# ska-sa/katsdpsigproc

Hardware: AMD Instinct MI355X
Metric: visibility samples/s (baselines x channels) through full RFI flagger (higher is better)
Workload: dtype f32 amplitude / f64 deviations

## Files before the change

### include/katsdpsigproc_hip.h

```cpp
#ifndef KATSDPSIGPROC_HIP_H
#define KATSDPSIGPROC_HIP_H

#include <stddef.h>
#include <stdint.h>

#ifdef __cplusplus
extern "C" {
#endif

#define KSP_ABI_VERSION 5

#define KSP_FLAGS_NONE 0
#define KSP_FLAGS_CHANNEL 1
#define KSP_FLAGS_FULL 2

#define KSP_THRESHOLD_SIMPLE 0
#define KSP_THRESHOLD_SUM 1

#define KSP_MAX_WINDOWS 8

typedef struct ksp_device_props {
    char name[256];
    char arch[64];
    int32_t compute_units;
// ... 31 lines not shown
int ksp_memcpy_async(int device, void *dst, const void *src, size_t bytes, int kind,
                     void *stream);
int ksp_memcpy_rect_async(int device, void *dst, size_t dst_origin, const size_t dst_strides[3],
                          const void *src, size_t src_origin, const size_t src_strides[3],
                          const size_t shape[3], int ndim, int kind, void *stream);
int ksp_memset_async(int device, void *ptr, int value, size_t bytes, void *stream);


int ksp_transpose(int device, void *stream, void *dst, const void *src, int in_rows, int in_cols,
                  int out_stride, int in_stride, int elem_size);

int ksp_percentile5_float(int device, void *stream, const void *in, float *out, int rows,
                          int in_stride, int out_stride, int first_col, int n_cols,
                          int is_amplitude);

int ksp_maskedsum_float(int device, void *stream, const void *in, const float *mask, void *out,
                        int in_stride, int n_rows, int n_cols, int use_amplitudes);

int ksp_background_median_filter(int device, void *stream, const void *in, float *out,
                                 const uint8_t *flags, int channels, int baselines, int stride,
                                 int flags_stride, int width, int is_amplitude, int flags_mode,
                                 int csplit);

int ksp_background_median_filter_geometry(int channels, int baselines, int width, int csplit,
                                          int *seg_len, int *n_segs);

int ksp_madnz_t(int device, void *stream, const float *in, float *noise, int channels,
                int baselines, int stride);

int ksp_madnz(int device, void *stream, const float *in, float *noise, int channels,
              int baselines, int stride);

int ksp_threshold_simple(int device, void *stream, const float *deviations, const float *noise,
                         uint8_t *flags, int rows, int cols, int stride, float n_sigma,
                         int flag_value, int transposed);

int ksp_threshold_sum(int device, void *stream, const float *deviations, const float *noise,
                      uint8_t *flags, int channels, int baselines, int stride, float n_sigma,
                      const float *scales, int n_windows, int flag_value, int vt);

int ksp_threshold_sum_cm(int device, void *stream, const float *deviations, const float *noise,
                         uint8_t *flags, int channels, int baselines, int stride, float n_sigma,
                         const float *scales, int n_windows, int flag_value);

int ksp_flagger_fused(int device, void *stream, const void *vis, const uint8_t *in_flags,
                      uint8_t *flags, float *deviations, float *noise, int channels,
                      int baselines, int vis_stride, int in_flags_stride, int flags_stride,
                      int dev_stride, int width, int is_amplitude, int flags_mode,
                      int threshold_kind, double n_sigma, const double *scales64, int n_windows,
                      int flag_value, void *workspace);

int ksp_flagger_fused_profile(void *start_event, void *stop_event);

int ksp_flagger_fused_supported(int channels, int width, int n_windows);

#define KSP_FUSED_PATH_STRIP 1
#define KSP_FUSED_PATH_LONG 2
#define KSP_FUSED_PATH_RING 4
int ksp_flagger_fused_last_path(void);

int ksp_flagger_fused_ring_mode(int mode);

int ksp_selftest_sqrt12(int device, void *stream, float *out, int n);
int ksp_selftest_abs(int device, void *stream, const float *re, const float *im, float *out,
                     int n);

int ksp_selftest_rank(int device, void *stream, const float *data, int *out, int n, int m);
int ksp_selftest_minmax(int device, void *stream, const float *data, float *out, int n);
int ksp_selftest_median_non_zero(int device, void *stream, const float *data, float *out,
                                 int n);

int ksp_rtc_compile(int device, const char *source, const char *const *options, int n_options,
                    void **module_out, char *log, size_t log_capacity);
int ksp_module_get_function(int device, void *module, const char *name, void **function_out);
int ksp_module_unload(int device, void *module);
int ksp_launch_function(int device, void *stream, void *function, const unsigned *grid,
                        const unsigned *block, unsigned shared_bytes, void **kernel_params);

#define KSP_FFT_R2C 0x2a
#define KSP_FFT_C2R 0x2c
#define KSP_FFT_C2C 0x29
#define KSP_FFT_D2Z 0x6a
#define KSP_FFT_Z2D 0x6c
#define KSP_FFT_Z2Z 0x69
int ksp_fft_plan_create(int device, int rank, const long long *n, const long long *inembed,
                        long long idist, const long long *onembed, long long odist, int type,
                        long long batch, void **plan_out, size_t *work_size);
int ksp_fft_plan_destroy(int device, void *plan);
int ksp_fft_exec(int device, void *stream, void *plan, int type, void *src, void *dest,
                 void *work_area, int inverse);

#define KSP_TDF_MAX_TIME 4096
#define KSP_TDF_MAX_FREQ 65536
#define KSP_TDF_MAX_WINDOWS 32
#define KSP_TDF_MAX_CHUNKS 512
#define KSP_TDF_MAX_RADIUS 2047
typedef struct ksp_twodflag_params {
    int n_time, n_freq, average_freq, is_amplitude;
    int n_windows_time, n_windows_freq;
    int windows_time[KSP_TDF_MAX_WINDOWS], windows_freq[KSP_TDF_MAX_WINDOWS];
    double tf_time[KSP_TDF_MAX_WINDOWS], tf_freq[KSP_TDF_MAX_WINDOWS];
    int n_chunks;
    int chunk_ends[KSP_TDF_MAX_CHUNKS + 1];
    int background_iterations, time_extend, freq_extend;
    double spike_width_time, spike_width_freq;
    double threshold_scale, reject_scale, flag_all_time_frac, flag_all_freq_frac;
} ksp_twodflag_params;
int ksp_twodflag_workspace(const ksp_twodflag_params *params, int batch, size_t *bytes);
typedef struct ksp_twodflag_offsets {
    size_t spec_flags, spec_background, spec_residual, spec_st;
    size_t flags, background, residual, time_flags, freq_flags, combined;
    size_t row_flags, row_all, col_all;
} ksp_twodflag_offsets;
int ksp_twodflag_layout(const ksp_twodflag_params *params, int batch, ksp_twodflag_offsets *out);
int ksp_twodflag(int device, void *stream, const void *data, const uint8_t *in_flags,
// ... 113 lines not shown
```

### katsdpsigproc_amd/_lib.py

```python

import contextlib
import ctypes
import os
import sys
from ctypes import POINTER, byref, c_char_p, c_double, c_float, c_int, c_int32, c_int64, c_size_t
from ctypes import c_void_p

_HERE = os.path.dirname(os.path.abspath(__file__))
LIB_PATH = os.path.join(_HERE, "_native", "libkatsdpsigproc_hip.so")
ABI_VERSION = 5

FUSED_PATH_STRIP = 1
FUSED_PATH_LONG = 2
FUSED_PATH_RING = 4

_lib = None


class DeviceProps(ctypes.Structure):

    _fields_ = [
        ("name", ctypes.c_char * 256),
        ("arch", ctypes.c_char * 64),
        ("compute_units", c_int32),
# ... 17 lines not shown

    _fields_ = [
        ("n_time", c_int), ("n_freq", c_int), ("average_freq", c_int), ("is_amplitude", c_int),
        ("n_windows_time", c_int), ("n_windows_freq", c_int),
        ("windows_time", c_int * TDF_MAX_WINDOWS), ("windows_freq", c_int * TDF_MAX_WINDOWS),
        ("tf_time", c_double * TDF_MAX_WINDOWS), ("tf_freq", c_double * TDF_MAX_WINDOWS),
        ("n_chunks", c_int), ("chunk_ends", c_int * (TDF_MAX_CHUNKS + 1)),
        ("background_iterations", c_int), ("time_extend", c_int), ("freq_extend", c_int),
        ("spike_width_time", c_double), ("spike_width_freq", c_double),
        ("threshold_scale", c_double), ("reject_scale", c_double),
        ("flag_all_time_frac", c_double), ("flag_all_freq_frac", c_double),
    ]


class TwodflagOffsets(ctypes.Structure):

    _fields_ = [(name, c_size_t) for name in (
        "spec_flags", "spec_background", "spec_residual", "spec_st", "flags", "background",
        "residual", "time_flags", "freq_flags", "combined", "row_flags", "row_all", "col_all",
    )]


SIGNATURES = {
    "ksp_device_count": [POINTER(c_int)],
    "ksp_device_get_props": [c_int, POINTER(DeviceProps)],
    "ksp_malloc": [c_int, c_size_t, POINTER(c_void_p)],
    "ksp_free": [c_int, c_void_p],
    "ksp_host_alloc": [c_size_t, POINTER(c_void_p)],
    "ksp_host_free": [c_void_p],
    "ksp_stream_create": [c_int, POINTER(c_void_p)],
    "ksp_stream_destroy": [c_int, c_void_p],
    "ksp_stream_synchronize": [c_int, c_void_p],
    "ksp_event_create": [c_int, POINTER(c_void_p)],
    "ksp_event_create_ordering": [c_int, POINTER(c_void_p)],
    "ksp_event_destroy": [c_int, c_void_p],
    "ksp_event_record": [c_int, c_void_p, c_void_p],
    "ksp_event_synchronize": [c_int, c_void_p],
    "ksp_event_elapsed_ms": [c_int, c_void_p, c_void_p, POINTER(c_float)],
    "ksp_stream_wait_event": [c_int, c_void_p, c_void_p],
    "ksp_memcpy_async": [c_int, c_void_p, c_void_p, c_size_t, c_int, c_void_p],
    "ksp_memcpy_rect_async": [
        c_int, c_void_p, c_size_t, POINTER(c_size_t), c_void_p, c_size_t, POINTER(c_size_t),
        POINTER(c_size_t), c_int, c_int, c_void_p,
    ],
    "ksp_memset_async": [c_int, c_void_p, c_int, c_size_t, c_void_p],
    "ksp_transpose": [c_int, c_void_p, c_void_p, c_void_p, c_int, c_int, c_int, c_int, c_int],
    "ksp_percentile5_float": [
        c_int, c_void_p, c_void_p, c_void_p, c_int, c_int, c_int, c_int, c_int, c_int
    ],
    "ksp_maskedsum_float": [
        c_int, c_void_p, c_void_p, c_void_p, c_void_p, c_int, c_int, c_int, c_int
    ],
    "ksp_flagger_fused_profile": [c_void_p, c_void_p],
    "ksp_selftest_sqrt12": [c_int, c_void_p, c_void_p, c_int],
    "ksp_selftest_abs": [c_int, c_void_p, c_void_p, c_void_p, c_void_p, c_int],
    "ksp_selftest_rank": [c_int, c_void_p, c_void_p, c_void_p, c_int, c_int],
    "ksp_selftest_minmax": [c_int, c_void_p, c_void_p, c_void_p, c_int],
    "ksp_selftest_median_non_zero": [c_int, c_void_p, c_void_p, c_void_p, c_int],
    "ksp_background_median_filter": [
        c_int, c_void_p, c_void_p, c_void_p, c_void_p, c_int, c_int, c_int, c_int, c_int, c_int,
        c_int, c_int,
    ],
    "ksp_background_median_filter_geometry": [
        c_int, c_int, c_int, c_int, POINTER(c_int), POINTER(c_int)
    ],
    "ksp_madnz_t": [c_int, c_void_p, c_void_p, c_void_p, c_int, c_int, c_int],
    "ksp_madnz": [c_int, c_void_p, c_void_p, c_void_p, c_int, c_int, c_int],
    "ksp_threshold_simple": [
        c_int, c_void_p, c_void_p, c_void_p, c_void_p, c_int, c_int, c_int, c_float, c_int, c_int
    ],
    "ksp_threshold_sum": [
        c_int, c_void_p, c_void_p, c_void_p, c_void_p, c_int, c_int, c_int, c_float,
        POINTER(c_float), c_int, c_int, c_int,
    ],
    "ksp_threshold_sum_cm": [
        c_int, c_void_p, c_void_p, c_void_p, c_void_p, c_int, c_int, c_int, c_float,
        POINTER(c_float), c_int, c_int,
    ],
    "ksp_flagger_fused": [
        c_int, c_void_p, c_void_p, c_void_p, c_void_p, c_void_p, c_void_p, c_int, c_int, c_int,
        c_int, c_int, c_int, c_int, c_int, c_int, c_int, c_double, POINTER(c_double), c_int,
        c_int, c_void_p,
    ],
    "ksp_flagger_fused_supported": [c_int, c_int, c_int],
    "ksp_flagger_fused_last_path": [],
    "ksp_flagger_fused_ring_mode": [c_int],
    "ksp_rtc_compile": [
        c_int, c_char_p, POINTER(c_char_p), c_int, POINTER(c_void_p), c_char_p, c_size_t
    ],
    "ksp_module_get_function": [c_int, c_void_p, c_char_p, POINTER(c_void_p)],
    "ksp_module_unload": [c_int, c_void_p],
    "ksp_fft_plan_create": [
        c_int, c_int, POINTER(ctypes.c_longlong), POINTER(ctypes.c_longlong), ctypes.c_longlong,
        POINTER(ctypes.c_longlong), ctypes.c_longlong, c_int, ctypes.c_longlong,
        POINTER(c_void_p), POINTER(c_size_t),
    ],
    "ksp_fft_plan_destroy": [c_int, c_void_p],
    "ksp_fft_exec": [c_int, c_void_p, c_void_p, c_int, c_void_p, c_void_p, c_void_p, c_int],
    "ksp_twodflag_workspace": [POINTER(TwodflagParams), c_int, POINTER(c_size_t)],
    "ksp_twodflag_layout": [POINTER(TwodflagParams), c_int, POINTER(TwodflagOffsets)],
    "ksp_twodflag": [
        c_int, c_void_p, c_void_p, c_void_p, c_void_p, c_int, ctypes.c_longlong, ctypes.c_longlong,
        c_int, c_int, POINTER(TwodflagParams), c_void_p, c_size_t,
    ],
    "ksp_masked_filter_workspace": [
        c_int, c_int, c_int, c_int, c_int, c_int, c_int, POINTER(c_size_t),
# ... 150 lines not shown
```

### katsdpsigproc_amd/csrc/flagger_fused.hip

```cpp
#include "flagger_fused_kernel.h"

static thread_local hipEvent_t g_prof_start = nullptr, g_prof_stop = nullptr;
static thread_local int g_last_path = 0;

__global__ __launch_bounds__(256) void fused_zero_rows_kernel(uint8_t *__restrict__ base, int rows,
                                                              int cols, size_t stride, int pieces)
{
    const size_t gid = (size_t)blockIdx.x * 256 + threadIdx.x;
    const size_t row = gid / (unsigned)pieces;
    if (row >= (size_t)rows) return;
    const int k = (int)(gid - row * (unsigned)pieces);
    const uintptr_t begin = (uintptr_t)base + row * stride, end = begin + (uintptr_t)cols;
    const uintptr_t piece = (begin & ~(uintptr_t)15) + 16 * (uintptr_t)k;
    if (piece >= end) return;
    if (piece >= begin && piece + 16 <= end) {
        *(uint4 *)piece = make_uint4(0u, 0u, 0u, 0u);
    } else {
        const uintptr_t lo = piece > begin ? piece : begin;
        const uintptr_t hi = piece + 16 < end ? piece + 16 : end;
        for (uintptr_t a = lo; a < hi; a++) *(uint8_t *)a = 0;
    }
}

hipError_t fused_zero_flags(const FusedParams &p, hipStream_t s)
{
    if (p.flags_stride == p.baselines)
        return hipMemsetAsync(p.flags, 0, (size_t)p.channels * p.baselines, s);
    const int pieces = (p.baselines + 15) / 16 + 1;
    const size_t lanes = (size_t)p.channels * pieces;
    hipLaunchKernelGGL(fused_zero_rows_kernel, dim3((unsigned)((lanes + 255) / 256)), dim3(256), 0, s,
                       p.flags, p.channels, p.baselines, (size_t)p.flags_stride, pieces);
    return hipGetLastError();
}

extern "C" int ksp_flagger_fused_profile(void *start_event, void *stop_event)
{
    KSP_REQUIRE((start_event == nullptr) == (stop_event == nullptr), "need both events or none");
    g_prof_start = (hipEvent_t)start_event;
    g_prof_stop = (hipEvent_t)stop_event;
    return 0;
}

extern "C" int ksp_flagger_fused_last_path(void) { return g_last_path; }

static thread_local int g_ring_mode = 2;
static int ring_mode()
{
    if (g_ring_mode == 2) {
        const char *e = getenv("KSP_FUSED_RING");
        g_ring_mode = e == nullptr ? 0 : (e[0] == '1' ? 1 : -1);
    }
    return g_ring_mode;
}
extern "C" int ksp_flagger_fused_ring_mode(int mode)
{
    const int before = ring_mode();
    if (mode >= -1 && mode <= 1) g_ring_mode = mode;
    return before;
}

extern "C" int ksp_flagger_fused_supported(int channels, int width, int n_windows)
{
    if (n_windows < 1 || n_windows > KSP_MAX_WINDOWS) return 0;
    if (channels > 4096) return n_windows <= 4 && ksp_fused_long_supported(channels, width);
    return channels >= 1 && width >= 3 && width <= 31 && (width & 1);
}

static int check_fused_args(const void *vis, const uint8_t *in_flags, const uint8_t *flags,
                            const float *deviations, int channels, int baselines, int vis_stride,
                            int in_flags_stride, int flags_stride, int dev_stride, int width,
                            int flags_mode, int threshold_kind, const double *scales64,
                            int &n_windows)
{
    KSP_REQUIRE(vis != nullptr && flags != nullptr, "NULL buffer");
    KSP_REQUIRE(channels >= 1 && baselines >= 0, "bad shape");
    KSP_REQUIRE(vis_stride >= baselines && flags_stride >= baselines, "stride smaller than row");
    KSP_REQUIRE(deviations == nullptr || dev_stride >= baselines, "bad dev_stride");
    KSP_REQUIRE(flags_mode >= KSP_FLAGS_NONE && flags_mode <= KSP_FLAGS_FULL, "bad flags_mode");
    KSP_REQUIRE(flags_mode == KSP_FLAGS_NONE || in_flags != nullptr, "in_flags is NULL");
    KSP_REQUIRE(flags_mode != KSP_FLAGS_FULL || in_flags_stride >= baselines, "bad in_flags_stride");
    KSP_REQUIRE(threshold_kind == KSP_THRESHOLD_SIMPLE || threshold_kind == KSP_THRESHOLD_SUM,
                "bad threshold_kind");
    KSP_REQUIRE(threshold_kind == KSP_THRESHOLD_SIMPLE || scales64 != nullptr, "scales64 is NULL");
    if (threshold_kind == KSP_THRESHOLD_SIMPLE && n_windows < 1) n_windows = 1;
    if (!ksp_flagger_fused_supported(channels, width, n_windows)) {
        ksp_set_error("ksp_flagger_fused: unsupported configuration (channels=%d width=%d "
                      "n_windows=%d); use the per-stage kernels", channels, width, n_windows);
        return (int)hipErrorNotSupported;
    }
    KSP_REQUIRE((vis_stride & 1) == 0, "vis_stride must be even");
    KSP_REQUIRE(((uintptr_t)vis & 15) == 0, "vis must be 16-byte aligned");
    return 0;
}

static void set_schedule(FusedParams &p, bool have_workspace)
{
// ... 46 lines not shown
    FusedParams t = p;
    t.vis = (const float2 *)p.vis + first;
    t.flags = p.flags + first;
    if (p.noise != nullptr) t.noise = p.noise + first;
    t.baselines = count;
    set_schedule(t, false);
    return t;
}

struct FusedPath {
    int bits, lanes, tail;
};

static FusedPath choose_path(const FusedParams &p, int width, int n_cu, int mode)
{
    const bool want_ring = mode != 0 ? mode > 0 : p.baselines / 8 >= 4 * n_cu;
    if (want_ring && width == 13 && ksp_ring_supported(p, width)) {
        const int tail = p.baselines % 8;
        return {KSP_FUSED_PATH_RING | (tail != 0 ? KSP_FUSED_PATH_STRIP : 0), 64, tail};
    }
    if (p.channels > 4096) return {KSP_FUSED_PATH_LONG, 64, 0};
    const bool wide = p.threshold_kind == KSP_THRESHOLD_SUM && p.n_windows > 4;
    if (width != 13 || wide || p.channels > 64 * 16) return {KSP_FUSED_PATH_STRIP, 64, 0};
    return {KSP_FUSED_PATH_STRIP, p.channels <= 64 * 4 ? 4 : 16, 0};
}

static int launch_strip(int lanes, int width, int device, hipStream_t s, const FusedParams &p,
                        hipEvent_t ev0, hipEvent_t ev1)
{
    if (width == 13) {
        if (lanes == 64) return launch_fused<64, 13>(device, s, p, ev0, ev1);
        if (lanes == 4) return launch_fused<4, 13>(device, s, p, ev0, ev1);
        return launch_fused<16, 13>(device, s, p, ev0, ev1);
    }
    int rc = 0;
    if (ksp_dispatch_exact<3, 5, 7, 9, 11, 15, 17, 19, 21, 23, 25, 27, 29, 31>(width, [&](auto W) {
            rc = ksp_fused_launch_width<W()>(device, s, p, ev0, ev1);
        }))
        return rc;
    ksp_set_error("fused flagger: width %d is not compiled here", width);
    return (int)hipErrorInvalidValue;
}

extern "C" int ksp_flagger_fused(int device, void *stream, const void *vis,
                                 const uint8_t *in_flags, uint8_t *flags, float *deviations,
                                 float *noise, int channels, int baselines, int vis_stride,
                                 int in_flags_stride, int flags_stride, int dev_stride, int width,
                                 int is_amplitude, int flags_mode, int threshold_kind,
                                 double n_sigma, const double *scales64, int n_windows,
                                 int flag_value, void *workspace)
{
    const hipEvent_t ev0 = g_prof_start, ev1 = g_prof_stop;
    g_prof_start = g_prof_stop = nullptr;
    g_last_path = 0;
    int rc = check_fused_args(vis, in_flags, flags, deviations, channels, baselines, vis_stride,
                              in_flags_stride, flags_stride, dev_stride, width, flags_mode,
                              threshold_kind, scales64, n_windows);
    if (rc != 0 || baselines == 0) return rc;
    KSP_CHECK(hipSetDevice(device));
    static KspPerDevice<int> cus;
    int n_cu = cus.get(device);
    if (n_cu == 0) {
        KSP_CHECK(hipDeviceGetAttribute(&n_cu, hipDeviceAttributeMultiprocessorCount, device));
        cus.set(device, n_cu);
    }
    const FusedParams p = make_params(vis, in_flags, flags, deviations, noise, channels, baselines,
                                      vis_stride, in_flags_stride, flags_stride, dev_stride,
                                      is_amplitude, flags_mode, threshold_kind, n_sigma, scales64,
                                      n_windows, flag_value, workspace, n_cu);
    hipStream_t s = (hipStream_t)stream;
    const FusedPath path = choose_path(p, width, n_cu, ring_mode());
    if (path.bits & KSP_FUSED_PATH_RING) {
        KSP_CHECK(fused_zero_flags(p, s));
        if (path.tail != 0) {
            const FusedParams t = columns(p, baselines - path.tail, path.tail);
            rc = launch_fused<64, 13>(device, s, t, nullptr, nullptr, false);
            if (rc != 0) return rc;
            g_last_path |= KSP_FUSED_PATH_STRIP;
        }
        g_last_path |= KSP_FUSED_PATH_RING;
        return ksp_ring_launch(width, device, s, p, n_cu, ev0, ev1);
    }
    g_last_path = path.bits;
    if (path.bits == KSP_FUSED_PATH_LONG) return ksp_fused_launch_long(device, s, p, ev0, ev1);
    return launch_strip(path.lanes, width, device, s, p, ev0, ev1);
}
```

### katsdpsigproc_amd/csrc/fused_common.h

```cpp
#pragma once
#include <stdlib.h>

#include "bitplane.h"
#include "median_merge.h"
#include "median_window.h"

#ifndef FUSED_MAD_BITS
#define FUSED_MAD_BITS 1
#endif
#ifndef FUSED_STRIP
#define FUSED_STRIP 4
#endif
#define FUSED_THREADS (64 * FUSED_STRIP)
#define FUSED_MAD_NORMAL 1.4826

#ifdef KSP_DIAG_REALTIME
#define FUSED_DIAG_CLOCK() __builtin_amdgcn_s_memrealtime()
#else
#define FUSED_DIAG_CLOCK() __builtin_amdgcn_s_memtime()
#endif
#ifdef KSP_DIAG
#define FUSED_DIAG_STOP(p) ((p).debug_stop)
#define FUSED_DIAG_TRACE(p) ((p).trace)
#else
#define FUSED_DIAG_STOP(p) 0
#define FUSED_DIAG_TRACE(p) ((unsigned long long *)nullptr)
#endif

struct FusedParams {
    const void *vis;
    const uint8_t *in_flags;
    uint8_t *flags;
    float *deviations;
    float *noise;
    int channels, baselines;
    int vis_stride, in_flags_stride, flags_stride, dev_stride;
    int is_amplitude, flags_mode, threshold_kind, n_windows, flag_value;
    int n_strips;
    int n_static, n_dyn, dyn_blocks;
    unsigned *work;
    int first_round;
#ifdef KSP_DIAG
    int debug_stop;
    unsigned long long *trace;
#endif
    double n_sigma;
    double scales[KSP_MAX_WINDOWS];
};

template <int R>
struct FusedLayout {
    static constexpr int RUN = R + 4;
    static constexpr int ROW = 64 * RUN + 8;
    static constexpr int LDS_FLOATS = FUSED_STRIP * ROW;
    static constexpr int LIST_DOUBLES = 256;
    static constexpr size_t LDS_BYTES =
        sizeof(float) * LDS_FLOATS + sizeof(double) * LIST_DOUBLES * FUSED_STRIP;
    __device__ static __forceinline__ int index(int c) { return (c / R) * RUN + (c % R); }
};

#ifndef FUSED_XCD_GROUP
#define FUSED_XCD_GROUP 8
#endif
__device__ __forceinline__ int strip_of(int id, int n_strips)
{
    constexpr int G = FUSED_XCD_GROUP;
    const int full = (n_strips / (8 * G)) * (8 * G);
    if (id >= full) return id;
    const int xcd = id & 7, i = id >> 3;
    return ((i / G) * 8 + xcd) * G + (i % G);
}

__device__ __forceinline__ float amp_with_flags(const FusedParams &p, float re, float im,
                                                int row, int bl)
{
    float a = ksp_abs_c64(re, im);
    if (p.flags_mode == KSP_FLAGS_CHANNEL) {
        if (p.in_flags[row]) a = __builtin_nanf("");
    } else if (p.flags_mode == KSP_FLAGS_FULL) {
        if (p.in_flags[(size_t)row * p.in_flags_stride + bl]) a = __builtin_nanf("");
    }
    return a;
}

template <int R>
__device__ __forceinline__ void load_strip(const FusedParams &p, float *lds, int b0, int tid)
{
// ... 1233 lines not shown
```

### katsdpsigproc_amd/csrc/fused_dispatch.h

```cpp
#pragma once
#include "fused_common.h"

hipError_t fused_zero_flags(const FusedParams &p, hipStream_t s);

template <int WIDTH>
int ksp_fused_launch_width(int device, hipStream_t s, const FusedParams &p, hipEvent_t ev0,
                           hipEvent_t ev1);

int ksp_fused_long_supported(int channels, int width);
int ksp_fused_launch_long(int device, hipStream_t s, const FusedParams &p, hipEvent_t ev0,
                          hipEvent_t ev1);
int ksp_fused_launch_long3(int device, hipStream_t s, const FusedParams &p, hipEvent_t ev0,
                           hipEvent_t ev1);

bool ksp_ring_supported(const FusedParams &p, int width);
int ksp_ring_launch(int width, int device, hipStream_t s, const FusedParams &p, int n_cu,
                    hipEvent_t ev0, hipEvent_t ev1);
```

### katsdpsigproc_amd/csrc/ring_kernel.h

```cpp
#pragma once
#include "fused_dispatch.h"
#include "launch.h"

#ifndef RING_STOP
#define RING_STOP 0
#endif
#define RING_THREADS 512
#define RING_STRIP 8
#define RING_NSLOT 32
#ifndef RING_G
#define RING_G 4
#endif
#ifndef RING_PRIO
#define RING_PRIO 0
#endif
#ifndef RING_STAGGER
#define RING_STAGGER 0
#endif
#define RING_SLOT_BYTES 4096
#define RING_LIST_DOUBLES 256
#define RING_XCD_GROUP 8

struct RingLayout {
    static constexpr size_t RING_BYTES = (size_t)RING_NSLOT * RING_SLOT_BYTES;
// ... 415 lines not shown
        unsigned long long exact;
        {
            const unsigned ra = __builtin_bitreverse32(ex_a), rb = __builtin_bitreverse32(ex_b);
            exact = ((unsigned long long)ra << H) |
                    ((unsigned long long)(rb & ((1u << (32 - H)) - 1u)) << (H + 32)) |
                    (unsigned long long)(rb >> (32 - H));
            unsigned long long first_odd = 0, last_odd = 0;
#pragma unroll
            for (int j = 0; j < H; j++)
                if ((H - j) & 1) first_odd |= 1ull << j;
#pragma unroll
            for (int j = R - H; j < R; j++)
                if ((j + H - R + 1) & 1) last_odd |= 1ull << j;
            if (lane == 0) exact &= ~first_odd;
            if (lane == 63) exact &= ~last_odd;
        }
        if (ksp_any(umax >= 0x7f800000u)) {
            float a2[R + 2 * H];
            int c_first = lane * R - H;
            asm volatile("" : "+v"(c_first));
#pragma unroll
            for (int i = 0; i < R + 2 * H; i++) a2[i] = fetch(c_first + i);
            tiny = 0;
            median_phase_src<R, W>([&](int i) { return a2[i + H]; }, dev, dmax, &tiny);
            exact = 0;
        }
        const bool ticket = more && k_strip + 2 >= p.n_static;
        unsigned t_own = 0;
        if (tid == 0 && ticket) t_own = atomicAdd(&p.work[RING_WORK_LIST + xcd], 1u);

#if RING_STOP == 1 || RING_STOP == 2
        {
            float acc = dmax;
#pragma unroll
            for (int j = 0; j < R; j++) acc += dev[j];
            if (acc == 12345.678f && p.noise != nullptr) p.noise[bl] = acc;
        }
#else
        const double noise64 = mad_noise<R, W, RING_LIST_DOUBLES, true>(dev, lane, list, fetch, RING_STOP > 30 ? RING_STOP : 0,
#ifdef RING_TRACE
                                                                      (trace_it < RING_TRACE_STRIPS && blockIdx.x < 256)
                                                                          ? &ring_trace_buf[((blockIdx.x * 8 + wave) * RING_TRACE_STRIPS + trace_it) * RING_TRACE_SLOTS]
                                                                          : nullptr,
#else
                                                                      nullptr,
#endif
                                                                      exact, &mad_hint, tiny);
        if (lane == 0 && p.noise != nullptr) p.noise[bl] = (float)noise64;
        RING_STAMP(2);
#if RING_STOP == 3 || RING_STOP > 30
        if (noise64 == 12345.678 && p.noise != nullptr) p.noise[bl] = dmax;
#else
        const unsigned long long fl = threshold_flags<R, W>(p, dev, dmax, noise64, lane, C, fetch);
        write_flags(p, fl, lane * R, bl, C);
        RING_STAMP(3);
#endif
#endif

#ifdef RING_TRACE
        if (lane_id == 0 && trace_it < RING_TRACE_STRIPS && blockIdx.x < 256)
            ring_trace_buf[((blockIdx.x * 8 + wave) * RING_TRACE_STRIPS + trace_it) * RING_TRACE_SLOTS + 7] = (unsigned long long)cur + 1;
        trace_it++;
#endif
        if (!more) break;
        cur = nxt;
        if (!ticket) {
            nxt = static_strip(k_strip + 2);
#ifdef RING_END_SYNC
            __syncthreads();
#endif
        } else {
            if (tid == 0) {
                int take = ring_strip_of(xcd, t0 + (int)t_own);
                if (take >= p.n_strips) take = ring_take(p.work, (xcd + 1) & 7, p.n_strips, t0);
                ctrl[2] = take;
            }
            __syncthreads();
            nxt = __builtin_amdgcn_readfirstlane(ctrl[2]);
            __syncthreads();
        }
        k_strip++;
    }
    finish();
}

inline bool ring_supported(const FusedParams &p, int width)
{
    return p.channels == 4096 && width % 2 == 1 && width >= 3 && width <= 13 && !p.is_amplitude &&
           p.flags_mode == KSP_FLAGS_NONE && p.deviations == nullptr && p.work != nullptr &&
           p.baselines >= RING_STRIP && (p.vis_stride % 2) == 0 &&
           (p.threshold_kind != KSP_THRESHOLD_SUM || p.n_windows <= 4) &&
           (size_t)p.vis_stride * 8 * 4096 < 0x7fffff00ull;
}

template <int WIDTH>
inline int launch_ring(int device, hipStream_t s, const FusedParams &p_in, int n_cu, hipEvent_t ev0,
                       hipEvent_t ev1)
{
    FusedParams p = p_in;
    p.n_strips = p.baselines / RING_STRIP;
    auto kern = flagger_ring_kernel<WIDTH>;
    int rc = ksp_lds_opt_in<flagger_ring_kernel<WIDTH>>(device, RingLayout::LDS_BYTES);
    if (rc != 0) return rc;
    const int grid = p.n_strips < n_cu ? p.n_strips : n_cu;
    p.n_static = 0;
    if (grid % 8 == 0 && p.n_strips / grid >= 3) {
        const int by_share = p.n_strips / grid - 2;
// ... 32 lines not shown
```

### katsdpsigproc_amd/hip.py

```python

import ctypes
import weakref
from typing import Any, List, Optional, Sequence, Tuple

import numpy as np

from . import _lib
from .abc import (
    AbstractCommandQueue,
    AbstractContext,
    AbstractDevice,
    AbstractEvent,
    AbstractKernel,
    AbstractProgram,
    AbstractTuningCommandQueue,
)

_H2D, _D2H, _D2D = 0, 1, 2


def _size3(values: Sequence[int]):
    padded = list(values) + [1] * (3 - len(values))
    return (ctypes.c_size_t * 3)(*padded)

# ... 317 lines not shown
        if not 1 <= ndim <= 3:
            raise ValueError("rect copies support 1 to 3 dimensions")
        _lib.call(
            "ksp_memcpy_rect_async", self._dev, ctypes.c_void_p(dst_ptr), int(dst_origin),
            _size3(dst_strides), ctypes.c_void_p(src_ptr), int(src_origin), _size3(src_strides),
            _size3(shape), ndim, kind, self._s
        )

    def enqueue_copy_buffer_rect(
        self, src_buffer, dest_buffer, src_origin, dest_origin, shape, src_strides, dest_strides
    ) -> None:
        self._rect(dest_buffer.ptr, dest_origin, dest_strides, src_buffer.ptr, src_origin,
                   src_strides, shape, _D2D)

    def enqueue_read_buffer_rect(
        self, buffer, data, buffer_origin, data_origin, shape, buffer_strides, data_strides,
        blocking: bool = True,
    ) -> None:
        self._rect(data.ctypes.data, data_origin, data_strides, buffer.ptr, buffer_origin,
                   buffer_strides, shape, _D2H)
        self._after_copy(data, blocking)

    def enqueue_write_buffer_rect(
        self, buffer, data, buffer_origin, data_origin, shape, buffer_strides, data_strides,
        blocking: bool = True,
    ) -> None:
        self._rect(buffer.ptr, buffer_origin, buffer_strides, data.ctypes.data, data_origin,
                   data_strides, shape, _H2D)
        self._after_copy(data, blocking)

    def enqueue_zero_buffer(self, buffer: Buffer) -> None:
        _lib.call("ksp_memset_async", self._dev, ctypes.c_void_p(buffer.ptr), 0, buffer.nbytes,
                  self._s)

    def enqueue_kernel(self, kernel, args, global_size=None, local_size=None) -> None:
        if isinstance(kernel, RtcKernel):
            self._enqueue_rtc(kernel, args, global_size, local_size)
            return
        if not isinstance(kernel, NativeKernel):
            raise TypeError("not a kernel of the HIP backend")
        converted = []
        for arg in args:
            if isinstance(arg, Buffer):
                converted.append(ctypes.c_void_p(arg.ptr))
            elif arg is None:
                converted.append(ctypes.c_void_p(0))
            elif isinstance(arg, (np.integer, np.bool_)):
                converted.append(int(arg))
            elif isinstance(arg, np.floating):
                converted.append(float(arg))
            else:
                converted.append(arg)
        _lib.call(kernel.name, self._dev, self._s, *converted)

    _CTYPES = {
        np.dtype(np.int8): ctypes.c_int8, np.dtype(np.uint8): ctypes.c_uint8,
        np.dtype(np.int16): ctypes.c_int16, np.dtype(np.uint16): ctypes.c_uint16,
        np.dtype(np.int32): ctypes.c_int32, np.dtype(np.uint32): ctypes.c_uint32,
        np.dtype(np.int64): ctypes.c_int64, np.dtype(np.uint64): ctypes.c_uint64,
        np.dtype(np.float32): ctypes.c_float, np.dtype(np.float64): ctypes.c_double,
        np.dtype(np.bool_): ctypes.c_bool,
    }

    def _enqueue_rtc(self, kernel: RtcKernel, args, global_size, local_size) -> None:
        if global_size is None or local_size is None:
            raise ValueError("global_size and local_size are required for compiled kernels")
        if len(global_size) != len(local_size) or not 1 <= len(global_size) <= 3:
            raise ValueError("global_size and local_size must have 1 to 3 dimensions each")
        grid, block = [], []
        for g, l in zip(global_size, local_size):
            if l <= 0 or g % l != 0:
                raise ValueError("global size is not a multiple of the local size")
            grid.append(g // l)
            block.append(l)
        if any(n == 0 for n in grid):
            return
        grid += [1] * (3 - len(grid))
        block += [1] * (3 - len(block))
        values = []
        for arg in args:
            if isinstance(arg, Buffer):
                values.append(ctypes.c_void_p(arg.ptr))
            elif isinstance(arg, RawBuffer):
                values.append(ctypes.c_void_p(arg.ptr))
            elif arg is None:
                values.append(ctypes.c_void_p(0))
            elif isinstance(arg, np.generic):
                if arg.dtype == np.complex64:
                    values.append((ctypes.c_float * 2)(arg.real, arg.imag))
                elif arg.dtype == np.complex128:
                    values.append((ctypes.c_double * 2)(arg.real, arg.imag))
                elif arg.dtype in self._CTYPES:
                    values.append(self._CTYPES[arg.dtype](arg.item()))
                else:
                    raise TypeError(f"cannot pass a {arg.dtype} scalar to a kernel")
            else:
                raise TypeError(
                    f"kernel argument {arg!r} is neither a device buffer nor a numpy scalar "
                    "(plain Python numbers have no definite C type)"
                )
        params = (ctypes.c_void_p * max(1, len(values)))(
            *[ctypes.cast(ctypes.pointer(v), ctypes.c_void_p) for v in values]
        )
        _lib.call("ksp_launch_function", self._dev, self._s, ctypes.c_void_p(kernel.handle),
                  (ctypes.c_uint * 3)(*grid), (ctypes.c_uint * 3)(*block), 0, params)

# ... 45 lines not shown
```

### katsdpsigproc_amd/rfi/device.py

```python

import ctypes
from abc import ABC, abstractmethod
from typing import Any, List, Mapping, Optional, Tuple, Type, Union

import numpy as np

from .. import _lib, _native_op, accel, transpose, tune
from ..abc import AbstractCommandQueue, AbstractContext
from ..accel import AbstractAllocator
from . import BackgroundFlags, host

_THRESHOLD_SUM_DEFAULT_THRESHOLD_FALLOFF = 1.2


def ctypes_float_array(values):
    return (ctypes.c_float * len(values))(*[float(v) for v in values])


def ctypes_double_array(values):
    return (ctypes.c_double * len(values))(*[float(v) for v in values])


def _check_shape(channels: int, baselines: int) -> None:
    if channels < 1 or baselines < 1:
# ... 631 lines not shown
        )


class FlaggerDevice(accel.OperationSequence):

    def __init__(self, template: FlaggerDeviceTemplate, command_queue: AbstractCommandQueue,
                 channels: int, baselines: int, background_args: Mapping[str, Any] = {},
                 noise_est_args: Mapping[str, Any] = {}, threshold_args: Mapping[str, Any] = {},
                 allocator: Optional[AbstractAllocator] = None) -> None:
        self.template = template
        self.channels = channels
        self.baselines = baselines
        self.background = template.background.instantiate(
            command_queue, channels, baselines, allocator=allocator, **background_args
        )
        self.noise_est = template.noise_est.instantiate(
            command_queue, channels, baselines, allocator=allocator, **noise_est_args
        )
        self.threshold = template.threshold.instantiate(
            command_queue, channels, baselines, allocator=allocator, **threshold_args
        )
        stages: List[Tuple[str, accel.Operation]] = [("background", self.background)]
        if template.transpose_deviations is not None:
            self.transpose_deviations = template.transpose_deviations.instantiate(
                command_queue, (channels, baselines)
            )
            stages.append(("transpose_deviations", self.transpose_deviations))
        stages.append(("noise_est", self.noise_est))
        stages.append(("threshold", self.threshold))
        if template.transpose_flags is not None:
            self.transpose_flags = template.transpose_flags.instantiate(
                command_queue, (baselines, channels)
            )
            stages.append(("transpose_flags", self.transpose_flags))

        dev_of_noise = "deviations_t" if self.noise_est.transposed else "deviations"
        dev_of_threshold = "deviations_t" if self.threshold.transposed else "deviations"
        flags_of_threshold = "flags_t" if self.threshold.transposed else "flags"
        compounds = {
            "vis": ["background:vis"],
            "input_flags": ["background:flags"],
            "deviations": ["background:deviations", "transpose_deviations:src"],
            "deviations_t": ["transpose_deviations:dest"],
            "noise": ["noise_est:noise", "threshold:noise"],
            "flags_t": ["transpose_flags:src"],
            "flags": ["transpose_flags:dest"],
        }
        compounds[dev_of_noise].append("noise_est:deviations")
        compounds[dev_of_threshold].append("threshold:deviations")
        compounds[flags_of_threshold].append("threshold:flags")
        super().__init__(command_queue, stages, compounds, allocator=allocator)


class FusedFlaggerDevice(accel.Operation):

    _OPTIONAL = ("deviations", "deviations_t", "flags_t")

    def __init__(self, template: FlaggerDeviceTemplate, command_queue: AbstractCommandQueue,
                 channels: int, baselines: int, threshold_args: Mapping[str, Any] = {},
                 allocator: Optional[AbstractAllocator] = None, vis_pad: int = 0) -> None:
        super().__init__(command_queue, allocator)
        if vis_pad < 0 or vis_pad % 2:
            raise ValueError("vis_pad must be even and not negative")
        self.template = template
        self.kernel = template._fused_kernel
        self.channels = channels
        self.baselines = baselines
        bg = template.background
        th = template.threshold
        args = dict(threshold_args)
        if "n_sigma" not in args:
            raise TypeError("threshold_args must provide n_sigma")
        self.n_sigma = float(args.pop("n_sigma"))
        if isinstance(th, ThresholdSumDeviceTemplate):
            falloff = float(args.pop("threshold_falloff", _THRESHOLD_SUM_DEFAULT_THRESHOLD_FALLOFF))
            self.threshold_kind = 1
            self.n_windows = th.n_windows
            self.scales = ctypes_double_array([pow(falloff, -i) for i in range(th.n_windows)])
        else:
            self.threshold_kind = 0
            self.n_windows = 1
            self.scales = ctypes_double_array([1.0])
        if args:
            raise TypeError(f"unexpected threshold arguments {sorted(args)}")
        vis_type = np.float32 if bg.is_amplitude else np.complex64
        self.vis_pad = vis_pad
        self.slots["vis"] = accel.IOSlot(
            (channels, accel.Dimension(baselines, min_padded_size=baselines + vis_pad, alignment=2)),
            vis_type,
        )
        if bg.use_flags == BackgroundFlags.FULL:
            self.slots["input_flags"] = accel.IOSlot((channels, accel.Dimension(baselines)), np.uint8)
        elif bg.use_flags == BackgroundFlags.CHANNEL:
            self.slots["input_flags"] = accel.IOSlot((channels,), np.uint8)
        self.slots["noise"] = accel.IOSlot((baselines,), np.float32)
        context = command_queue.context
        self._transpose_dev = transpose.TransposeTemplate(context, np.float32, "float").instantiate(
            command_queue, (channels, baselines), allocator=allocator)
        self._transpose_flags = transpose.TransposeTemplate(
            context, np.uint8, "unsigned char").instantiate(
            command_queue, (channels, baselines), allocator=allocator)
        self.slots["flags"] = accel.CompoundIOSlot([
            accel.IOSlot((channels, accel.Dimension(baselines)), np.uint8),
            self._transpose_flags.slots["src"]])
        self.slots["deviations"] = accel.CompoundIOSlot([
            accel.IOSlot((channels, accel.Dimension(baselines)), np.float32),
            self._transpose_dev.slots["src"]])
        self.slots["deviations_t"] = self._transpose_dev.slots["dest"]
        self.slots["flags_t"] = self._transpose_flags.slots["dest"]
        self._mandatory = [name for name in self.slots
                           if name not in self._OPTIONAL
                           or (name == "deviations" and template.keep_deviations)]
        self._workspace = accel.DeviceArray(command_queue.context, (16,), np.uint32)
        self._workspace.zero(command_queue)
        self._armed = None

    def ensure_all_bound(self) -> None:
        for name in self._mandatory:
            self.ensure_bound(name)

    def buffer(self, name: str) -> accel.DeviceArray:
        if name in self._OPTIONAL and not self.slots[name].is_bound():
            self.ensure_bound(name)
        return super().buffer(name)

    def required_bytes(self) -> int:
        return sum(slot.required_bytes() for name, slot in self.slots.items()
                   if name in self._mandatory or slot.is_bound())

    def _run(self) -> None:
        bg = self.template.background
        vis = self.buffer("vis")
        flags = self.buffer("flags")
        in_flags = self.buffer("input_flags") if bg.use_flags else None
        want_dev_t = self.slots["deviations_t"].is_bound()
        if want_dev_t:
            self.ensure_bound("deviations")
        dev = super().buffer("deviations") if self.slots["deviations"].is_bound() else None
        in_flags_stride = in_flags.padded_shape[1] if bg.use_flags == BackgroundFlags.FULL else 0
        self.command_queue.enqueue_kernel(
            self.kernel,
            [
                vis.buffer,
                in_flags.buffer if in_flags is not None else None,
                flags.buffer,
                dev.buffer if dev is not None else None,
                self.buffer("noise").buffer,
                np.int32(self.channels),
                np.int32(self.baselines),
                np.int32(vis.padded_shape[1]),
                np.int32(in_flags_stride),
                np.int32(flags.padded_shape[1]),
                np.int32(dev.padded_shape[1] if dev is not None else 0),
                np.int32(bg.width),
                np.int32(bg.is_amplitude),
                np.int32(bg.use_flags.value),
                np.int32(self.threshold_kind),
                float(self.n_sigma),
                self.scales,
                np.int32(self.n_windows),
                np.int32(self.template.threshold.flag_value),
                self._workspace.buffer,
            ],
        )
        self._armed = None
        if want_dev_t:
            self._transpose_dev()
        if self.slots["flags_t"].is_bound():
            self._transpose_flags()

    def profile_next_run(self):
        queue = self.command_queue
        start, stop = queue.create_event(), queue.create_event()
        _lib.call("ksp_flagger_fused_profile", ctypes.c_void_p(start.handle),
                  ctypes.c_void_p(stop.handle))
        self._armed = (start, stop)
        return start, stop

    def parameters(self) -> Mapping[str, Any]:
        return {
            "fused": True,
            "vis_pad": self.vis_pad,
            "keep_deviations": self.slots["deviations"].is_bound(),
            "width": self.template.background.width,
            "n_sigma": self.n_sigma,
            "n_windows": self.n_windows,
            "channels": self.channels,
            "baselines": self.baselines,
        }


class FlaggerHostFromDevice(host.AbstractFlaggerHost):
# ... 333 lines not shown
```

Before: 383.8 billion.

## Write ring-path flags as bitmasks and expand them in a separate kernel

On the ring path, the kernel can now store each baseline's 64-bit threshold flag mask into a scratch buffer instead of scattering byte flags into the output array. A new expand kernel then byte-permutes those masks into vectorised 16-byte flag stores, with a row-wise fallback for unaligned columns. When masks are used, the upfront zeroing of the flags array is skipped except for the tail columns. The cost is an extra kernel launch plus a round trip through the mask buffer. It is enabled only for a narrow configuration: 4096 channels, complex input, no input flags, width 13, and deviations not kept.

```diff
diff --git a/include/katsdpsigproc_hip.h b/include/katsdpsigproc_hip.h
--- a/include/katsdpsigproc_hip.h
+++ b/include/katsdpsigproc_hip.h
@@ -107,6 +107,8 @@
 
 int ksp_flagger_fused_profile(void *start_event, void *stop_event);
 
+int ksp_flagger_fused_flag_masks(void *scratch, size_t bytes);
+
 int ksp_flagger_fused_supported(int channels, int width, int n_windows);
 
 #define KSP_FUSED_PATH_STRIP 1
@@ -116,6 +118,8 @@
 
 int ksp_flagger_fused_ring_mode(int mode);
 
+int ksp_selftest_flag_expand(int device, void *stream, const void *masks, uint8_t *flags,
+                             int channels, int columns, int flags_stride, int flag_value);
 int ksp_selftest_sqrt12(int device, void *stream, float *out, int n);
 int ksp_selftest_abs(int device, void *stream, const float *re, const float *im, float *out,
                      int n);
diff --git a/katsdpsigproc_amd/_lib.py b/katsdpsigproc_amd/_lib.py
--- a/katsdpsigproc_amd/_lib.py
+++ b/katsdpsigproc_amd/_lib.py
@@ -93,6 +93,8 @@
         c_int, c_void_p, c_void_p, c_void_p, c_void_p, c_int, c_int, c_int, c_int
     ],
     "ksp_flagger_fused_profile": [c_void_p, c_void_p],
+    "ksp_flagger_fused_flag_masks": [c_void_p, c_size_t],
+    "ksp_selftest_flag_expand": [c_int, c_void_p, c_void_p, c_void_p, c_int, c_int, c_int, c_int],
     "ksp_selftest_sqrt12": [c_int, c_void_p, c_void_p, c_int],
     "ksp_selftest_abs": [c_int, c_void_p, c_void_p, c_void_p, c_void_p, c_int],
     "ksp_selftest_rank": [c_int, c_void_p, c_void_p, c_void_p, c_int, c_int],
diff --git a/katsdpsigproc_amd/csrc/flag_expand.hip b/katsdpsigproc_amd/csrc/flag_expand.hip
--- /dev/null
+++ b/katsdpsigproc_amd/csrc/flag_expand.hip
@@ -0,0 +1,141 @@
+#include "fused_dispatch.h"
+
+#define EXPAND_GROUPS 8
+#define EXPAND_COLS (16 * EXPAND_GROUPS)
+#define EXPAND_UNITS (256 / EXPAND_GROUPS)
+#define EXPAND_PIPE 2
+
+__device__ __forceinline__ void expand_transpose4(const unsigned *x, unsigned *out)
+{
+    const unsigned y0 = __builtin_amdgcn_perm(x[1], x[0], 0x05010400u);
+    const unsigned y1 = __builtin_amdgcn_perm(x[1], x[0], 0x07030602u);
+    const unsigned z0 = __builtin_amdgcn_perm(x[3], x[2], 0x05010400u);
+    const unsigned z1 = __builtin_amdgcn_perm(x[3], x[2], 0x07030602u);
+    out[0] = __builtin_amdgcn_perm(z0, y0, 0x05040100u);
+    out[1] = __builtin_amdgcn_perm(z0, y0, 0x07060302u);
+    out[2] = __builtin_amdgcn_perm(z1, y1, 0x05040100u);
+    out[3] = __builtin_amdgcn_perm(z1, y1, 0x07060302u);
+}
+
+template <bool FV1, bool WHOLE>
+__global__ __launch_bounds__(256) void flag_expand_kernel(const unsigned *__restrict__ masks,
+                                                          uint8_t *__restrict__ flags, int rows,
+                                                          int cols16, size_t stride, unsigned fv)
+{
+    const int t = threadIdx.x;
+    const int b = blockIdx.x * EXPAND_COLS + (t % EXPAND_GROUPS) * 16;
+    const int u0 = blockIdx.y * EXPAND_UNITS + t / EXPAND_GROUPS;
+    if (b >= cols16) return;
+    unsigned m[EXPAND_PIPE][16];
+#pragma unroll
+    for (int q = 0; q < EXPAND_PIPE; q++) {
+        const int u = u0 + q * (int)gridDim.y * EXPAND_UNITS;
+        if (u * 32 < rows) {
+#pragma unroll
+            for (int k = 0; k < 16; k++) {
+                m[q][k] = masks[(size_t)(b + k) * 128 + u];
+            }
+        }
+    }
+#pragma unroll
+    for (int q = 0; q < EXPAND_PIPE; q++) {
+        const int u = u0 + q * (int)gridDim.y * EXPAND_UNITS;
+        if (u * 32 >= rows) continue;
+        uint8_t *dst = flags + (size_t)u * 32 * stride + b;
+        const int n = rows - u * 32;
+#pragma unroll
+        for (int r = 0; r < 8; r++) {
+            unsigned v[4][4];
+#pragma unroll
+            for (int g = 0; g < 4; g++) {
+                unsigned x[4], y[4];
+#pragma unroll
+                for (int c = 0; c < 4; c++) x[c] = (m[q][4 * g + c] >> r) & 0x01010101u;
+                expand_transpose4(x, y);
+#pragma unroll
+                for (int i = 0; i < 4; i++) v[i][g] = FV1 ? y[i] : y[i] * fv;
+            }
+#pragma unroll
+            for (int i = 0; i < 4; i++) {
+                if (WHOLE || r + 8 * i < n) {
+                    uint8_t *to = dst + (size_t)(r + 8 * i) * stride;
+                    *(uint4 *)to = make_uint4(v[i][0], v[i][1], v[i][2], v[i][3]);
+                }
+            }
+        }
+    }
+}
+
+__global__ __launch_bounds__(256) void flag_expand_rows_kernel(
+    const unsigned long long *__restrict__ masks, uint8_t *__restrict__ flags, int rows, int col0,
+    int cols, size_t stride, int pieces, unsigned fv)
+{
+    const size_t gid = (size_t)blockIdx.x * 256 + threadIdx.x;
+    const size_t row = gid / (unsigned)pieces;
+    if (row >= (size_t)rows) return;
+    const int k = (int)(gid - row * (unsigned)pieces);
+    const uintptr_t begin = (uintptr_t)flags + row * stride + (uintptr_t)col0;
+    const uintptr_t end = begin + (uintptr_t)cols;
+    const uintptr_t piece = (begin & ~(uintptr_t)15) + 16 * (uintptr_t)k;
+    if (piece >= end) return;
+    const unsigned long long *mrow = masks + (row >> 6);
+    const int shift = (int)(row & 63);
+    auto value = [&](uintptr_t a) -> unsigned {
+        const size_t b = (size_t)col0 + (size_t)(a - begin);
+        return ((mrow[b * 64] >> shift) & 1ull) ? fv : 0u;
+    };
+    if (piece >= begin && piece + 16 <= end) {
+        unsigned word[4];
+#pragma unroll
+        for (int i = 0; i < 4; i++) {
+            word[i] = 0;
+#pragma unroll
+            for (int q = 0; q < 4; q++) word[i] |= value(piece + 4 * i + q) << (8 * q);
+        }
+        *(uint4 *)piece = make_uint4(word[0], word[1], word[2], word[3]);
+    } else {
+        const uintptr_t lo = piece > begin ? piece : begin;
+        const uintptr_t hi = piece + 16 < end ? piece + 16 : end;
+        for (uintptr_t a = lo; a < hi; a++) *(uint8_t *)a = (uint8_t)value(a);
+    }
+}
+
+int ksp_fused_expand_flags(hipStream_t s, const unsigned long long *masks, uint8_t *flags,
+                           int channels, int cols, size_t stride, int flag_value)
+{
+    if (cols <= 0) return 0;
+    const unsigned fv = (unsigned)flag_value & 0xffu;
+    const bool aligned = ((uintptr_t)flags & 15) == 0 && (stride & 15) == 0;
+    const int cols16 = aligned ? cols & ~15 : 0;
+    if (cols16 != 0) {
+        const dim3 grid((unsigned)ksp_divup(cols16, EXPAND_COLS),
+                        (unsigned)ksp_divup(channels, 32 * EXPAND_UNITS * EXPAND_PIPE));
+        auto kern = flag_expand_kernel<false, false>;
+        if (channels % 32 == 0)
+            kern = fv == 1 ? flag_expand_kernel<true, true> : flag_expand_kernel<false, true>;
+        hipLaunchKernelGGL(kern, grid, dim3(256), 0, s, (const unsigned *)masks, flags, channels,
+                           cols16, stride, fv);
+        KSP_LAUNCH_CHECK();
+    }
+    if (cols16 < cols) {
+        const int rest = cols - cols16;
+        const int pieces = (rest + 15) / 16 + 1;
+        const size_t lanes = (size_t)channels * pieces;
+        hipLaunchKernelGGL(flag_expand_rows_kernel, dim3((unsigned)((lanes + 255) / 256)), dim3(256),
+                           0, s, masks, flags, channels, cols16, rest, stride, pieces, fv);
+        KSP_LAUNCH_CHECK();
+    }
+    return 0;
+}
+
+extern "C" int ksp_selftest_flag_expand(int device, void *stream, const void *masks, uint8_t *flags,
+                                        int channels, int columns, int flags_stride, int flag_value)
+{
+    KSP_REQUIRE(masks != nullptr && flags != nullptr, "NULL buffer");
+    KSP_REQUIRE(channels >= 1 && channels <= 4096 && columns >= 0, "bad shape");
+    KSP_REQUIRE(flags_stride >= columns, "stride smaller than row");
+    KSP_REQUIRE(((uintptr_t)masks & 7) == 0, "masks must be 8-byte aligned");
+    KSP_CHECK(hipSetDevice(device));
+    return ksp_fused_expand_flags((hipStream_t)stream, (const unsigned long long *)masks, flags,
+                                  channels, columns, (size_t)flags_stride, flag_value);
+}
diff --git a/katsdpsigproc_amd/csrc/flagger_fused.hip b/katsdpsigproc_amd/csrc/flagger_fused.hip
--- a/katsdpsigproc_amd/csrc/flagger_fused.hip
+++ b/katsdpsigproc_amd/csrc/flagger_fused.hip
@@ -42,6 +42,17 @@
 }
 
 extern "C" int ksp_flagger_fused_last_path(void) { return g_last_path; }
+
+static thread_local unsigned long long *g_masks = nullptr;
+static thread_local size_t g_mask_bytes = 0;
+
+extern "C" int ksp_flagger_fused_flag_masks(void *scratch, size_t bytes)
+{
+    KSP_REQUIRE(((uintptr_t)scratch & 7) == 0, "scratch must be 8-byte aligned");
+    g_masks = (unsigned long long *)scratch;
+    g_mask_bytes = scratch != nullptr ? bytes : 0;
+    return 0;
+}
 
 static thread_local int g_ring_mode = 2;
 static int ring_mode()
@@ -194,6 +205,10 @@
 {
     const hipEvent_t ev0 = g_prof_start, ev1 = g_prof_stop;
     g_prof_start = g_prof_stop = nullptr;
+    unsigned long long *const masks = g_masks;
+    const size_t mask_bytes = g_mask_bytes;
+    g_masks = nullptr;
+    g_mask_bytes = 0;
     g_last_path = 0;
     int rc = check_fused_args(vis, in_flags, flags, deviations, channels, baselines, vis_stride,
                               in_flags_stride, flags_stride, dev_stride, width, flags_mode,
@@ -213,15 +228,23 @@
     hipStream_t s = (hipStream_t)stream;
     const FusedPath path = choose_path(p, width, n_cu, ring_mode());
     if (path.bits & KSP_FUSED_PATH_RING) {
-        KSP_CHECK(fused_zero_flags(p, s));
+        const int ring_cols = baselines - path.tail;
+        FusedParams r = p;
+        if (masks != nullptr && mask_bytes / (64 * sizeof(unsigned long long)) >= (size_t)ring_cols)
+            r.flag_masks = masks;
+        if (r.flag_masks == nullptr) KSP_CHECK(fused_zero_flags(p, s));
         if (path.tail != 0) {
-            const FusedParams t = columns(p, baselines - path.tail, path.tail);
+            const FusedParams t = columns(p, ring_cols, path.tail);
+            if (r.flag_masks != nullptr) KSP_CHECK(fused_zero_flags(t, s));
             rc = launch_fused<64, 13>(device, s, t, nullptr, nullptr, false);
             if (rc != 0) return rc;
             g_last_path |= KSP_FUSED_PATH_STRIP;
         }
         g_last_path |= KSP_FUSED_PATH_RING;
-        return ksp_ring_launch(width, device, s, p, n_cu, ev0, ev1);
+        rc = ksp_ring_launch(width, device, s, r, n_cu, ev0, ev1);
+        if (rc != 0 || r.flag_masks == nullptr) return rc;
+        return ksp_fused_expand_flags(s, r.flag_masks, p.flags, channels, ring_cols,
+                                      (size_t)flags_stride, flag_value);
     }
     g_last_path = path.bits;
     if (path.bits == KSP_FUSED_PATH_LONG) return ksp_fused_launch_long(device, s, p, ev0, ev1);
diff --git a/katsdpsigproc_amd/csrc/fused_common.h b/katsdpsigproc_amd/csrc/fused_common.h
--- a/katsdpsigproc_amd/csrc/fused_common.h
+++ b/katsdpsigproc_amd/csrc/fused_common.h
@@ -33,6 +33,7 @@
     uint8_t *flags;
     float *deviations;
     float *noise;
+    unsigned long long *flag_masks;
     int channels, baselines;
     int vis_stride, in_flags_stride, flags_stride, dev_stride;
     int is_amplitude, flags_mode, threshold_kind, n_windows, flag_value;
diff --git a/katsdpsigproc_amd/csrc/fused_dispatch.h b/katsdpsigproc_amd/csrc/fused_dispatch.h
--- a/katsdpsigproc_amd/csrc/fused_dispatch.h
+++ b/katsdpsigproc_amd/csrc/fused_dispatch.h
@@ -2,6 +2,9 @@
 #include "fused_common.h"
 
 hipError_t fused_zero_flags(const FusedParams &p, hipStream_t s);
+
+int ksp_fused_expand_flags(hipStream_t s, const unsigned long long *masks, uint8_t *flags,
+                           int channels, int cols, size_t stride, int flag_value);
 
 template <int WIDTH>
 int ksp_fused_launch_width(int device, hipStream_t s, const FusedParams &p, hipEvent_t ev0,
diff --git a/katsdpsigproc_amd/csrc/ring_kernel.h b/katsdpsigproc_amd/csrc/ring_kernel.h
--- a/katsdpsigproc_amd/csrc/ring_kernel.h
+++ b/katsdpsigproc_amd/csrc/ring_kernel.h
@@ -491,7 +491,14 @@
         if (noise64 == 12345.678 && p.noise != nullptr) p.noise[bl] = dmax;
 #else
         const unsigned long long fl = threshold_flags<R, W>(p, dev, dmax, noise64, lane, C, fetch);
-        write_flags(p, fl, lane * R, bl, C);
+#ifdef RING_NOFLAGS
+        asm volatile("" ::"v"(fl));
+#else
+        if (p.flag_masks != nullptr)
+            p.flag_masks[(size_t)bl * 64 + lane] = fl;
+        else
+            write_flags(p, fl, lane * R, bl, C);
+#endif
         RING_STAMP(3);
 #endif
 #endif
diff --git a/katsdpsigproc_amd/hip.py b/katsdpsigproc_amd/hip.py
--- a/katsdpsigproc_amd/hip.py
+++ b/katsdpsigproc_amd/hip.py
@@ -393,6 +393,9 @@
             else:
                 converted.append(arg)
         _lib.call(kernel.name, self._dev, self._s, *converted)
+
+    def lend_fused_flag_masks(self, buffer: Buffer) -> None:
+        _lib.call("ksp_flagger_fused_flag_masks", ctypes.c_void_p(buffer.ptr), buffer.nbytes)
 
     _CTYPES = {
         np.dtype(np.int8): ctypes.c_int8, np.dtype(np.uint8): ctypes.c_uint8,
diff --git a/katsdpsigproc_amd/rfi/device.py b/katsdpsigproc_amd/rfi/device.py
--- a/katsdpsigproc_amd/rfi/device.py
+++ b/katsdpsigproc_amd/rfi/device.py
@@ -707,6 +707,10 @@
         super().__init__(command_queue, stages, compounds, allocator=allocator)
 
 
+def _fused_flag_mask_words(baselines: int) -> int:
+    return (baselines // 8) * 8 * 64
+
+
 class FusedFlaggerDevice(accel.Operation):
 
     _OPTIONAL = ("deviations", "deviations_t", "flags_t")
@@ -768,6 +772,13 @@
                            or (name == "deviations" and template.keep_deviations)]
         self._workspace = accel.DeviceArray(command_queue.context, (16,), np.uint32)
         self._workspace.zero(command_queue)
+        self._flag_masks = None
+        if (channels == 4096 and not bg.is_amplitude and bg.use_flags == BackgroundFlags.NONE
+                and not template.keep_deviations and bg.width == 13
+                and _fused_flag_mask_words(baselines) > 0
+                and hasattr(command_queue, "lend_fused_flag_masks")):
+            self._flag_masks = accel.DeviceArray(
+                command_queue.context, (_fused_flag_mask_words(baselines),), np.uint64)
         self._armed = None
 
     def ensure_all_bound(self) -> None:
@@ -793,6 +804,8 @@
             self.ensure_bound("deviations")
         dev = super().buffer("deviations") if self.slots["deviations"].is_bound() else None
         in_flags_stride = in_flags.padded_shape[1] if bg.use_flags == BackgroundFlags.FULL else 0
+        if self._flag_masks is not None and dev is None:
+            self.command_queue.lend_fused_flag_masks(self._flag_masks.buffer)
         self.command_queue.enqueue_kernel(
             self.kernel,
             [
```

Result: slower. 371.7 billion (-3.2%).
